# yui-mhcp/text_to_speech

Hardware: AMD Instinct MI355X
Metric: audio samples/sec (22.05 kHz WaveGlow vocoding, fp32) (higher is better)
Workload: dtype f32; 1 GPU; WaveGlow-only vocoding of precomputed 80x800 mel, batch 8 per GPU, fp32 (BASELINE.json configs[1]); batch_per_gpu=8, mel_frames=800, world_size=1, backend=single process, weights=seeded synthetic (rng 1234)

## Files before the change

text_to_speech_amd/csrc/wn_wino.hip:

```cpp
#include "engine.h"
#include "gemm_f32.h"

#include <algorithm>

using namespace ttsgemm;

namespace {
constexpr int C = 512;
constexpr int NPH = 32;
constexpr int KMEL = 320;
constexpr int KCONV = 3 * C;

__device__ __forceinline__ f32x4 x_at(const float* __restrict__ x, int ps, long long f, int df, int c, int PR, int BT, int T) {
    const f32x4 zero = {0.f, 0.f, 0.f, 0.f};
    if (f >= BT) return zero;
    const int carry = (ps >> 5) + df;
    const int t = (int)(f % T) + carry;
    if (t < 0 || t >= T) return zero;
    return *reinterpret_cast<const f32x4*>(x + ((long long)(ps & 31) * PR + f + carry) * C + c);
}


__device__ __forceinline__ int group_phase0(int gp, int d) { return (gp / d) * 4 * d + gp % d; }

__host__ __device__ __forceinline__ int frame_groups_per_utt(int T) { return (T + 15) / 16 * 4; }
__device__ __forceinline__ bool frame_group(int gf, int s, int BT, int T, int& b, int& t0) {
    const int G = frame_groups_per_utt(T);
    b = gf / G;
    const int g = gf % G;
    t0 = (g / s) * 4 * s + g % s;
    return (long long)b * T < BT && t0 < T;
}
__host__ __device__ __forceinline__ int mixed_groups_per_utt(int T) { return (T + 1) / 2; }
__device__ __forceinline__ bool mixed_group(int gm, int BT, int T, int& b, int& t0) {
    const int G = mixed_groups_per_utt(T);
    b = gm / G;
    t0 = 2 * (gm % G);
    return (long long)b * T < BT;
}
__device__ __forceinline__ f32x4 x_bt(const float* __restrict__ x, int p, int b, int t, int c, int PR, int T) {
    const f32x4 zero = {0.f, 0.f, 0.f, 0.f};
    if (t < 0 || t >= T) return zero;
    return *reinterpret_cast<const f32x4*>(x + ((long long)p * PR + (long long)b * T + t) * C + c);
}

__global__ void wino4_prepass_kernel(const float* __restrict__ x, float* __restrict__ U, int d, int PR, int BT, int T, long long Mq) {
    const long long idx = (long long)blockIdx.x * blockDim.x + threadIdx.x;
    if (idx >= Mq * (C / 4)) return;
    const long long mg = idx / (C / 4);
    const int c = (int)(idx % (C / 4)) * 4;
    f32x4 v[6];
    if (d == 16) {
        const int PRm = (int)(Mq / 16);
        const int p0 = (int)(mg / PRm);
        int b, t0;
        const bool ok = mixed_group(mg % PRm, BT, T, b, t0);
        const f32x4 zero = {0.f, 0.f, 0.f, 0.f};
#pragma unroll
        for (int i = 0; i < 6; ++i) {
            const int ps = p0 + 16 * (i - 1);
            v[i] = ok ? x_bt(x, ps & 31, b, t0 + (ps >> 5), c, PR, T) : zero;
        }
    } else if (d < NPH) {
        const int gp = (int)(mg / PR);
        const long long f = mg % PR;
        const int p0 = group_phase0(gp, d);
#pragma unroll
        for (int i = 0; i < 6; ++i) v[i] = x_at(x, p0 + (i - 1) * d, f, 0, c, PR, BT, T);
    } else {
        const int s = d / NPH, PRq = (int)(Mq / NPH);
        const int p = (int)(mg / PRq);
        int b, t0;
        const bool ok = frame_group(mg % PRq, s, BT, T, b, t0);
        const f32x4 zero = {0.f, 0.f, 0.f, 0.f};
#pragma unroll
        for (int i = 0; i < 6; ++i) v[i] = ok ? x_bt(x, p, b, t0 + (i - 1) * s, c, PR, T) : zero;
    }
    const long long o = mg * C + c, plane = Mq * C;
    *reinterpret_cast<f32x4*>(U + o) = 4.f * v[0] - 5.f * v[2] + v[4];
    *reinterpret_cast<f32x4*>(U + plane + o) = -4.f * (v[1] + v[2]) + v[3] + v[4];
    *reinterpret_cast<f32x4*>(U + 2 * plane + o) = 4.f * (v[1] - v[2]) - v[3] + v[4];
    *reinterpret_cast<f32x4*>(U + 3 * plane + o) = 2.f * (v[3] - v[1]) - v[2] + v[4];
    *reinterpret_cast<f32x4*>(U + 4 * plane + o) = 2.f * (v[1] - v[3]) - v[2] + v[4];
    *reinterpret_cast<f32x4*>(U + 5 * plane + o) = 4.f * v[1] - 5.f * v[3] + v[5];
}

__global__ void wino4_weights_kernel(const float* __restrict__ in_Bt, float* __restrict__ G) {
    const int idx = blockIdx.x * blockDim.x + threadIdx.x;
    if (idx >= 2 * C * C) return;
    const int n = idx / C, c = idx % C;
    const float* row = in_Bt + (long long)n * KCONV + (c / 16) * 48 + c % 16;
    const double wm = row[0], w0 = row[16], wp = row[32];
    const long long plane = (long long)2 * C * C;
    G[idx] = (float)(wm / 4.0);
    G[plane + idx] = (float)(-(wm + w0 + wp) / 6.0);
    G[2 * plane + idx] = (float)(-(wm - w0 + wp) / 6.0);
    G[3 * plane + idx] = (float)(wm / 24.0 + w0 / 12.0 + wp / 6.0);
    G[4 * plane + idx] = (float)(wm / 24.0 - w0 / 12.0 + wp / 6.0);
    G[5 * plane + idx] = (float)wp;
}

constexpr int NPT = 7, NMEL = 80;
__constant__ double C44_G[7][4] = {{1., 0., 0., 0.},
                                   {1., 1., 1., 1.},
                                   {1., -1., 1., -1.},
                                   {1., 2., 4., 8.},
                                   {1., -2., 4., -8.},
                                   {1., 1. / 2, 1. / 4, 1. / 8},
                                   {1., -1. / 2, 1. / 4, -1. / 8}};
__constant__ double C44_BT[7][7] = {{1., 0., -21. / 4, 0., 21. / 4, 0., -1.},
                                    {0., -2. / 9, -2. / 9, 17. / 18, 17. / 18, -2. / 9, -2. / 9},
                                    {0., 2. / 9, -2. / 9, -17. / 18, 17. / 18, 2. / 9, -2. / 9},
                                    {0., 1. / 180, 1. / 360, -1. / 36, -1. / 72, 1. / 45, 1. / 90},
                                    {0., -1. / 180, 1. / 360, 1. / 36, -1. / 72, -1. / 45, 1. / 90},
                                    {0., 64. / 45, 128. / 45, -16. / 9, -32. / 9, 16. / 45, 32. / 45},
                                    {0., -64. / 45, 128. / 45, 16. / 9, -32. / 9, -16. / 45, 32. / 45}};

constexpr int K4 = 224, SA = 112, SB = 96, SC = 112;
constexpr int KF = 160;
[[maybe_unused]] __constant__ double FIR_X[5] = {0, 1, -1, 2, -2};
[[maybe_unused]] __constant__ double FIR_BT[5][5] = {{1, 0, -5. / 4, 0, 1. / 4},
                                                     {0, 2. / 3, 2. / 3, -1. / 6, -1. / 6},
                                                     {0, -2. / 3, 2. / 3, 1. / 6, -1. / 6},
                                                     {0, -1. / 12, -1. / 24, 1. / 12, 1. / 24},
                                                     {0, 1. / 12, -1. / 24, -1. / 12, 1. / 24}};
__host__ __device__ __forceinline__ int fir_qb(int s, int half) { return s == 1 ? 2 * half + 1 : half + 2; }
struct InKernelCondChunks {
    unsigned long long cfg_lo = 0, cfg_hi = 0;
};
inline InKernelCondChunks in_kernel_cond_chunks(bool phases, bool mixed, bool fir) {
    InKernelCondChunks a;
    unsigned ccfg[6] = {0, 0, 0, 0, 0, 0};
    auto cc = [](unsigned n1, unsigned b1, unsigned n2 = 0, unsigned b2 = 0) { return n1 | b1 << 5 | n2 << 9 | b2 << 12; };
    if (phases) {
        for (int p = 0; p < 6; ++p) ccfg[p] = cc(p == 1 || p == 2 ? K4 / 16 : (SA + SB) / 16, 0);
    } else if (mixed) {
        for (int p = 1; p < 5; ++p) ccfg[p] = cc(KMEL / 16, 0);
    } else if (fir) {
        for (int p = 0; p < 5; ++p) ccfg[p] = cc(KF / 16, 0);
    } else {
        ccfg[0] = ccfg[5] = cc((SA + SB) / 16, 0);
        ccfg[1] = ccfg[2] = cc(SA / 16, 0, SC / 16, (SA + SB) / 16);
        ccfg[3] = ccfg[4] = cc((SB + SC) / 16, SA / 16);
    }
    for (int p = 0; p < 6; ++p) (p < 4 ? a.cfg_lo : a.cfg_hi) |= (unsigned long long)ccfg[p] << (16 * (p & 3));
    return a;
}

__host__ __device__ __forceinline__ int cond_groups_per_utt(int T) { return (T + 3) / 4; }

__global__ void wino_cond_weights_kernel(const float* __restrict__ cond_Bt, float* __restrict__ W) {
    const long long idx = (long long)blockIdx.x * blockDim.x + threadIdx.x;
    if (idx >= (long long)NPH * NPT * 2 * C * NMEL) return;
    const int c = (int)(idx % NMEL), n = (int)((idx / NMEL) % (2 * C)), x = (int)((idx / ((long long)NMEL * 2 * C)) % NPT),
              p = (int)(idx / ((long long)NMEL * 2 * C * NPT));
    const float* row = cond_Bt + ((long long)p * 2 * C + n) * KMEL + c;
    double acc = 0.0;
#pragma unroll
    for (int q = 0; q < 4; ++q) acc += C44_G[x][3 - q] * (double)row[q * NMEL];
    W[idx] = (float)acc;
}

__global__ void wino_cond_mel_planes_kernel(const float* __restrict__ mel, float* __restrict__ Z, int rows, int BT, int T) {
    const long long idx = (long long)blockIdx.x * blockDim.x + threadIdx.x;
    if (idx >= (long long)NPT * rows * NMEL) return;
    const int c = (int)(idx % NMEL), gr = (int)((idx / NMEL) % rows), x = (int)(idx / ((long long)rows * NMEL));
    const int G = cond_groups_per_utt(T), b = gr / G, t0 = 4 * (gr % G);
    double acc = 0.0;
    if ((long long)b * T < BT) {
#pragma unroll
        for (int i = 0; i < NPT; ++i) {
            const int t = t0 - 3 + i;
            if (t >= 0 && t < T) acc += C44_BT[x][i] * (double)mel[((long long)b * T + t) * NMEL + c];
        }
    }
    Z[idx] = (float)acc;
}

__global__ void wino_cond_rows_kernel(int* __restrict__ tab, int rows, int BT, int T) {
    const int gr = blockIdx.x * blockDim.x + threadIdx.x;
    if (gr >= rows) return;
    const int G = cond_groups_per_utt(T), b = gr / G, t0 = 4 * (gr % G);
    const int left = T - t0;
    tab[gr] = (long long)b * T < BT ? (b * T + t0) | (left < 4 ? left : 4) << 16 : 0;
}

struct WinoCondArgs {
    const float* Z;
    const int* rowtab;
    const float* W;
    const float* bias;
    float* cond;
    int rows;
    int PR, BT, T;
};

template <int WR, int WC, int NBUF, int OCC>
__global__ __launch_bounds__(WR * WC * 64, OCC) void wino_cond_kernel(const WinoCondArgs g) {
    constexpr int NW = WR * WC, BM = WR * 32, BN = WC * 32;
    constexpr int NPA = BM / 16, NPB = BN / 16, PPW = (NPA + NPB) / NW;
    static_assert((NPA + NPB) % NW == 0 && PPW <= 4, "the pieces of a tile divide among the waves, one per MFMA of a half step");
    constexpr int STAGE = (BM + BN) * 16;
    constexpr int NKC = NMEL / 16, NT = NPT * NKC;
    typedef __attribute__((address_space(3))) void* lds_ptr_t;
    extern __shared__ __attribute__((aligned(16))) float smem[];
    const int tid = threadIdx.x, lane = tid & 63;
    const int wave = __builtin_amdgcn_readfirstlane(tid >> 6);
    const int wr = wave / WC, wc = wave % WC;
    const int li = lane & 31, lh = lane >> 5;

    constexpr int numNt = 2 * C / BN;
    const int numMt = g.rows / BM;
    const int bid = blockIdx.x, xcd = bid & 7, slot = bid >> 3;
    const int pair = (slot / numMt) * 8 + xcd, mt = slot % numMt;
    const int ph = pair / numNt, nt = pair % numNt;
    const int m0 = mt * BM, n0 = nt * BN;

    f32x16 acc[NPT];
#pragma unroll
    for (int p = 0; p < NPT; ++p)
#pragma unroll
        for (int r = 0; r < 16; ++r) acc[p][r] = 0.f;

    const int prow = lane >> 2, chunk = (lane & 3) ^ ((lane >> 4) & 3);
    unsigned vo0[PPW];
#pragma unroll
    for (int i = 0; i < PPW; ++i) {
        const int q = wave * PPW + i;
        const int row = (q < NPA ? q : q - NPA) * 16 + prow;
        vo0[i] = (unsigned)((row * NMEL + chunk * 4) * 4);
    }
    const float* const abase = g.Z + (long long)m0 * NMEL;
    const float* const bbase = g.W + ((long long)ph * NPT * 2 * C + n0) * NMEL;
    const long long zplane = (long long)g.rows * NMEL, wplane = (long long)2 * C * NMEL;
    int lt = 0;
    unsigned vo[PPW], ko = 0;
    const float* pb[PPW];
    auto prepare = [&]() {
        const bool live = lt < NT;
        const int x = live ? lt / NKC : 0, kc = live ? lt % NKC : 0;
        ko = (unsigned)kc * 64u;
#pragma unroll
        for (int i = 0; i < PPW; ++i) {
            const bool isA = wave * PPW + i < NPA;
            pb[i] = isA ? abase + x * zplane : bbase + x * wplane;
            vo[i] = live ? vo0[i] : OOB;
        }
        ++lt;
    };
    auto issue_piece = [&](int i, int buf) {
        const unsigned voff = vo[i], koff = ko;
        const float* base = pb[i];
        __builtin_amdgcn_raw_ptr_buffer_load_lds(make_rsrc_uniform(base), (lds_ptr_t)(smem + buf * STAGE + (wave * PPW + i) * 256), 16,
                                                 voff, koff, 0, 0);
    };
    const int xr = (li >> 2) & 3;
    struct Frag {
        f32x4 a, b;
    };
    auto read_frag = [&](int buf, int k8, Frag& f) {
        const int koff = ((2 * k8 + lh) ^ xr) * 4;
        f.a = *reinterpret_cast<const f32x4*>(smem + buf * STAGE + (wr * 32 + li) * 16 + koff);
        f.b = *reinterpret_cast<const f32x4*>(smem + buf * STAGE + BM * 16 + (wc * 32 + li) * 16 + koff);
    };

#pragma unroll
    for (int b = 0; b < NBUF; ++b) {
        prepare();
#pragma unroll
        for (int i = 0; i < PPW; ++i) issue_piece(i, b);
    }
    asm volatile("s_waitcnt vmcnt(%0)" ::"n"(PPW * (NBUF - 1)) : "memory");
    __builtin_amdgcn_s_barrier();
    Frag f0, f1;
    read_frag(0, 0, f0);
    int buf = 0;
    static_for<NPT>([&](auto pc) {
        constexpr int P = decltype(pc)::value;
        for (int s = 0; s < NKC; ++s) {
            read_frag(buf, 1, f1);
            prepare();
#pragma unroll
            for (int kk = 0; kk < 4; ++kk) acc[P] = __builtin_amdgcn_mfma_f32_32x32x2f32(f0.a[kk], f0.b[kk], acc[P], 0, 0, 0);
            __builtin_amdgcn_sched_barrier(0);
            asm volatile("s_waitcnt vmcnt(%0) lgkmcnt(0)" ::"n"(PPW * (NBUF - 2)) : "memory");
            __builtin_amdgcn_s_barrier();
            const int bufn = buf == NBUF - 1 ? 0 : buf + 1;
            read_frag(bufn, 0, f0);
            __builtin_amdgcn_sched_barrier(0);
#pragma unroll
            for (int kk = 0; kk < 4; ++kk) {
                acc[P] = __builtin_amdgcn_mfma_f32_32x32x2f32(f1.a[kk], f1.b[kk], acc[P], 0, 0, 0);
                if (kk < PPW) {
                    issue_piece(kk, buf);
                    __builtin_amdgcn_sched_barrier(0);
                }
            }
            buf = bufn;
        }
    });
    asm volatile("s_waitcnt vmcnt(0)" ::: "memory");

    const float bv = g.bias[n0 + wc * 32 + li];
    const int* const rt = g.rowtab + m0 + wr * 32 + 4 * lh;
    const __amdgpu_buffer_rsrc_t ro = make_rsrc_uniform(g.cond + (long long)ph * g.PR * (2 * C) + n0 + wc * 32);
#pragma unroll
    for (int r = 0; r < 16; ++r) {
        const int info = rt[(r & 3) + 8 * (r >> 2)];
        const unsigned voff = ((unsigned)(info & 0xffff) * (2 * C) + li) * 4u;
        const int nout = info >> 16;
        const float s12 = acc[1][r] + acc[2][r], d12 = acc[1][r] - acc[2][r];
        const float s34 = acc[3][r] + acc[4][r], d34 = acc[3][r] - acc[4][r];
        const float s56 = acc[5][r] + acc[6][r], d56 = acc[5][r] - acc[6][r];
        float y[4];
        y[0] = acc[0][r] + s12 + s34 + s56 + bv;
        y[1] = d12 + 2.f * d34 + 0.5f * d56 + bv;
        y[2] = s12 + 4.f * s34 + 0.25f * s56 + bv;
        y[3] = d12 + 8.f * d34 + 0.125f * d56 + bv;
#pragma unroll
        for (int j = 0; j < 4; ++j)
            __builtin_amdgcn_raw_buffer_store_b32(__builtin_bit_cast(unsigned, y[j]), ro, j < nout ? voff : OOB, j * (2 * C * 4), 0);
    }
}

template <int WR, int WC, int NBUF, int OCC>
hipError_t launch_wino_cond(const WinoCondArgs& a, hipStream_t st) {
    constexpr int BM = WR * 32, BN = WC * 32;
    const size_t lds = (size_t)NBUF * (BM + BN) * 16 * sizeof(float);
    if (a.rows % BM != 0) return hipErrorInvalidValue;
    auto kern = wino_cond_kernel<WR, WC, NBUF, OCC>;
    static PerDeviceOnce attr_set;
    if (hipError_t e = set_max_dyn_lds_once((const void*)kern, lds, attr_set); e != hipSuccess) return e;
    hipLaunchKernelGGL(kern, dim3((unsigned)(NPH * (2 * C / BN) * (a.rows / BM))), dim3(WR * WC * 64), lds, st, a);
    return hipGetLastError();
}

__device__ __forceinline__ unsigned group_out_pack(int kind, int gl, int sfr, int BT, int T) {
    if (kind == 0) return (unsigned)gl | 15u << 20;
    int b, t0;
    const bool ok = kind == 1 ? frame_group(gl, sfr, BT, T, b, t0) : mixed_group(gl, BT, T, b, t0);
    if (!ok) return 0u;
    const int left = T - t0;
    return (unsigned)(b * T + t0) | (unsigned)(left < 15 ? left : 15) << 20;
}
__device__ __forceinline__ long long group_out_base(int kind, int ph, int j, int d, int PR, unsigned& jstep) {
    if (kind == 0) {
        jstep = 0;
        return (long long)(group_phase0(ph, d) + j * d) * PR;
    }
    if (kind == 1) {
        jstep = (unsigned)(j * (d / NPH));
        return (long long)ph * PR + j * (d / NPH);
    }
    jstep = (unsigned)(j >> 1);
    return (long long)(ph + 16 * (j & 1)) * PR + (j >> 1);
}

__global__ void wino4_combine_kernel(const float* __restrict__ P, const float* __restrict__ cond, float* __restrict__ acts, int d,
                                     int PR, int BT, int T, long long Mq) {
    const long long idx = (long long)blockIdx.x * blockDim.x + threadIdx.x;
    if (idx >= Mq * (C / 4)) return;
    const long long mg = idx / (C / 4);
    const int ch = (int)(idx % (C / 4)) * 4;
    const int col = (ch >> 5) * 64 + (ch & 31);
    const long long plane = Mq * 2 * C, o = mg * 2 * C + col;
    f32x4 a[6], b[6];
#pragma unroll
    for (int z = 0; z < 6; ++z) {
        a[z] = __builtin_nontemporal_load(reinterpret_cast<const f32x4*>(P + z * plane + o));
        b[z] = __builtin_nontemporal_load(reinterpret_cast<const f32x4*>(P + z * plane + o + 32));
    }
    const int kind = d == 16 ? 2 : d < NPH ? 0 : 1;
    const int prows = kind == 0 ? PR : (int)(Mq / (kind == 2 ? 16 : NPH));
    const int ph = (int)(mg / prows);
    const unsigned pack = group_out_pack(kind, (int)(mg % prows), d / NPH, BT, T);
#pragma unroll
    for (int j = 0; j < 4; ++j) {
        unsigned jstep;
        const long long row = group_out_base(kind, ph, j, d, PR, jstep) + (pack & 0xfffffu);
        if (jstep >= pack >> 20) break;
        const f32x4 ca = *reinterpret_cast<const f32x4*>(cond + row * (2 * C) + col);
        const f32x4 cb = *reinterpret_cast<const f32x4*>(cond + row * (2 * C) + col + 32);
        f32x4 t, s;
        if (j == 0) {
            t = a[0] + a[1] + a[2] + a[3] + a[4] + ca;
            s = b[0] + b[1] + b[2] + b[3] + b[4] + cb;
        } else if (j == 1) {
            t = a[1] - a[2] + 2.f * (a[3] - a[4]) + ca;
            s = b[1] - b[2] + 2.f * (b[3] - b[4]) + cb;
        } else if (j == 2) {
            t = a[1] + a[2] + 4.f * (a[3] + a[4]) + ca;
            s = b[1] + b[2] + 4.f * (b[3] + b[4]) + cb;
        } else {
            t = a[1] - a[2] + 8.f * (a[3] - a[4]) + a[5] + ca;
            s = b[1] - b[2] + 8.f * (b[3] - b[4]) + b[5] + cb;
        }
        f32x4 g;
#pragma unroll
        for (int k = 0; k < 4; ++k) g[k] = gate_tanh_sigmoid(t[k], s[k]);
        *reinterpret_cast<f32x4*>(acts + row * C + ch) = g;
    }
}

__device__ __forceinline__ void wino_gate_store(const f32x16 (&acc)[6][2], float* patch, const float* __restrict__ cond,
                                                float* __restrict__ acts, int kind, int d, int ph, int gl0, int col0, int PR, int BT,
                                                int T, int lane) {
    const int li = lane & 31, lh = lane >> 5, er = lane >> 3, ec4 = (lane & 7) * 4;
    const int sfr = d / NPH;
    const int ch0 = (col0 >> 6) * 32 + ec4;
    unsigned orow[16];
#pragma unroll
    for (int r = 0; r < 16; ++r) {
        orow[r] = group_out_pack(kind, gl0 + (r & 3) + 8 * (r >> 2) + 4 * lh, sfr, BT, T);
        __builtin_amdgcn_sched_barrier(0);
    }
    static_for<4>([&](auto jc) {
        constexpr int j = decltype(jc)::value;
        unsigned jstep;
        const long long jb = group_out_base(kind, ph, j, d, PR, jstep);
        const __amdgpu_buffer_rsrc_t rc = make_rsrc_uniform(cond + jb * (2 * C) + col0);
        constexpr int RB = j == 0 ? 8 : 16;
#pragma unroll
        for (int r0 = 0; r0 < 16; r0 += RB) {
            float ctv[RB], csv[RB];
#pragma unroll
            for (int rr = 0; rr < RB; ++rr) {
                const unsigned pk = orow[r0 + rr];
                const unsigned off = jstep < pk >> 20 ? ((pk & 0xfffffu) * (2 * C) + li) * 4u : OOB;
                ctv[rr] = __builtin_bit_cast(float, __builtin_amdgcn_raw_buffer_load_b32(rc, off, 0, 0));
                csv[rr] = __builtin_bit_cast(float, __builtin_amdgcn_raw_buffer_load_b32(rc, off, 128, 0));
            }
            __builtin_amdgcn_sched_barrier(0);
#pragma unroll
            for (int rr = 0; rr < RB; ++rr) {
                const int r = r0 + rr;
                const float ct = ctv[rr], cs = csv[rr];
                float tv, sv;
                if constexpr (j == 0) {
                    tv = acc[0][0][r] + acc[1][0][r] + acc[2][0][r] + acc[3][0][r] + acc[4][0][r] + ct;
                    sv = acc[0][1][r] + acc[1][1][r] + acc[2][1][r] + acc[3][1][r] + acc[4][1][r] + cs;
                } else if constexpr (j == 1) {
                    tv = acc[1][0][r] - acc[2][0][r] + 2.f * (acc[3][0][r] - acc[4][0][r]) + ct;
                    sv = acc[1][1][r] - acc[2][1][r] + 2.f * (acc[3][1][r] - acc[4][1][r]) + cs;
                } else if constexpr (j == 2) {
                    tv = acc[1][0][r] + acc[2][0][r] + 4.f * (acc[3][0][r] + acc[4][0][r]) + ct;
                    sv = acc[1][1][r] + acc[2][1][r] + 4.f * (acc[3][1][r] + acc[4][1][r]) + cs;
                } else {
                    tv = acc[1][0][r] - acc[2][0][r] + 8.f * (acc[3][0][r] - acc[4][0][r]) + acc[5][0][r] + ct;
                    sv = acc[1][1][r] - acc[2][1][r] + 8.f * (acc[3][1][r] - acc[4][1][r]) + acc[5][1][r] + cs;
                }
                patch[((r & 3) + 8 * (r >> 2) + 4 * lh) * 36 + li] = gate_tanh_sigmoid(tv, sv);
            }
        }
        asm volatile("s_waitcnt lgkmcnt(0)" ::: "memory");
#pragma unroll
        for (int qq = 0; qq < 4; ++qq) {
            const f32x4 v = *reinterpret_cast<const f32x4*>(patch + (er + 8 * qq) * 36 + ec4);
            const unsigned srow = group_out_pack(kind, gl0 + er + 8 * qq, sfr, BT, T);
            if (jstep < srow >> 20) *reinterpret_cast<f32x4*>(acts + (jb + (srow & 0xfffffu)) * C + ch0) = v;
        }
        asm volatile("s_waitcnt lgkmcnt(0)" ::: "memory");
    });
}

struct WinoFusedArgs {
    const float* U;   long long uplane;
    const float* G;   long long gplane;
    const float* cond;
    float* acts;
    int Mq, phase_rows;
    int kind;
    int d, PR, BT, T;
};

template <int WR, int WC, int NBUF, int OCC>
__global__ __launch_bounds__(WR * WC * 64, OCC) void wino4_fused_kernel(const WinoFusedArgs g) {
    constexpr int NW = WR * WC, BM = WR * 32, BN = WC * 64;
    constexpr int NPA = BM / 16, NPB = BN / 16, PPW = (NPA + NPB) / NW;
    static_assert((NPA + NPB) % NW == 0, "the pieces of a tile divide among the waves");
    constexpr int STAGE = (BM + BN) * 16;
    static_assert(NBUF * STAGE >= NW * 32 * 36, "the epilogue's transpose patches fit the pipeline buffers");
    typedef __attribute__((address_space(3))) void* lds_ptr_t;
    extern __shared__ __attribute__((aligned(16))) float smem[];
    const int tid = threadIdx.x, lane = tid & 63;
    const int wave = __builtin_amdgcn_readfirstlane(tid >> 6);
    const int wr = wave / WC, wc = wave % WC;
    const int li = lane & 31, lh = lane >> 5;

    constexpr int numNt = 2 * C / BN;
    const int numMt = g.Mq / BM;
    const int bid = blockIdx.x, xcd = bid & 7, slot = bid >> 3;
    const int mt = (slot / numNt) * 8 + xcd, nt = slot % numNt;
    if (mt >= numMt) return;
    const int m0 = mt * BM, n0 = nt * BN;
    const int ph = m0 / g.phase_rows, fr0 = m0 - ph * g.phase_rows;

    f32x16 acc[6][2];
#pragma unroll
    for (int p = 0; p < 6; ++p)
#pragma unroll
        for (int h = 0; h < 2; ++h)
#pragma unroll
            for (int r = 0; r < 16; ++r) acc[p][h][r] = 0.f;

    const int prow = lane >> 2, chunk = (lane & 3) ^ ((lane >> 4) & 3);
    unsigned vo0[PPW];
#pragma unroll
    for (int i = 0; i < PPW; ++i) {
        const int q = wave * PPW + i;
        const int row = (q < NPA ? q : q - NPA) * 16 + prow;
        vo0[i] = (unsigned)((row * C + chunk * 4) * 4);
    }
    int lp = 0, lkc = 0;
    unsigned vo[PPW], ko = 0;
    const float* pb[PPW];
    auto prepare = [&]() {
        const bool live = lp < 6;
        const int p = live ? lp : 0;
        ko = (unsigned)lkc * 64u;
#pragma unroll
        for (int i = 0; i < PPW; ++i) {
            const bool isA = wave * PPW + i < NPA;
            pb[i] = isA ? g.U + p * g.uplane + (long long)m0 * C : g.G + p * g.gplane + (long long)n0 * C;
            vo[i] = live ? vo0[i] : OOB;
        }
        if (live && ++lkc == C / 16) {
            lkc = 0;
            ++lp;
        }
    };
    auto issue_piece = [&](int i, int buf) {
        const unsigned voff = vo[i], koff = ko;
        const float* base = pb[i];
        __builtin_amdgcn_raw_ptr_buffer_load_lds(make_rsrc_uniform(base), (lds_ptr_t)(smem + buf * STAGE + (wave * PPW + i) * 256), 16,
                                                 voff, koff, 0, 0);
    };
    const int xr = (li >> 2) & 3;
    struct Frag {
        f32x4 a, b0, b1;
    };
    auto read_frag = [&](int buf, int k8, Frag& f) {
        const int koff = ((2 * k8 + lh) ^ xr) * 4;
        const float* a = smem + buf * STAGE + (wr * 32 + li) * 16 + koff;
        const float* b = smem + buf * STAGE + BM * 16 + (wc * 64 + li) * 16 + koff;
        f.a = *reinterpret_cast<const f32x4*>(a);
        f.b0 = *reinterpret_cast<const f32x4*>(b);
        f.b1 = *reinterpret_cast<const f32x4*>(b + 32 * 16);
    };

#pragma unroll
    for (int b = 0; b < NBUF; ++b) {
        prepare();
#pragma unroll
        for (int i = 0; i < PPW; ++i) issue_piece(i, b);
    }
    asm volatile("s_waitcnt vmcnt(%0)" ::"n"(PPW * (NBUF - 1)) : "memory");
    __builtin_amdgcn_s_barrier();
    Frag f0, f1;
    read_frag(0, 0, f0);
    int buf = 0;
    static_for<6>([&](auto pc) {
        constexpr int P = decltype(pc)::value;
        for (int s = 0; s < C / 16; ++s) {
            read_frag(buf, 1, f1);
            prepare();
#pragma unroll
            for (int kk = 0; kk < 4; ++kk) {
                acc[P][0] = __builtin_amdgcn_mfma_f32_32x32x2f32(f0.a[kk], f0.b0[kk], acc[P][0], 0, 0, 0);
                acc[P][1] = __builtin_amdgcn_mfma_f32_32x32x2f32(f0.a[kk], f0.b1[kk], acc[P][1], 0, 0, 0);
            }
            __builtin_amdgcn_sched_barrier(0);
            asm volatile("s_waitcnt vmcnt(%0) lgkmcnt(0)" ::"n"(PPW * (NBUF - 2)) : "memory");
            __builtin_amdgcn_s_barrier();
            const int bufn = buf == NBUF - 1 ? 0 : buf + 1;
            read_frag(bufn, 0, f0);
            __builtin_amdgcn_sched_barrier(0);
#pragma unroll
            for (int kk = 0; kk < 4; ++kk) {
                acc[P][0] = __builtin_amdgcn_mfma_f32_32x32x2f32(f1.a[kk], f1.b0[kk], acc[P][0], 0, 0, 0);
                acc[P][1] = __builtin_amdgcn_mfma_f32_32x32x2f32(f1.a[kk], f1.b1[kk], acc[P][1], 0, 0, 0);
                if (kk < PPW) {
                    issue_piece(kk, buf);
                    __builtin_amdgcn_sched_barrier(0);
                }
            }
            static_assert(PPW <= 4, "one DMA piece per MFMA pair of the second half");
            buf = bufn;
        }
    });
    asm volatile("s_waitcnt vmcnt(0)" ::: "memory");
    __builtin_amdgcn_s_barrier();

    wino_gate_store(acc, smem + wave * (32 * 36), g.cond, g.acts, g.kind, g.d, ph, fr0 + wr * 32, n0 + wc * 64, g.PR, g.BT, g.T, lane);
}

template <int WR, int WC, int NBUF, int OCC>
hipError_t launch_wino_fused(const WinoFusedArgs& a, hipStream_t st) {
    constexpr int BM = WR * 32, BN = WC * 64;
    const size_t lds = (size_t)NBUF * (BM + BN) * 16 * sizeof(float);
    if (a.Mq % BM != 0 || a.phase_rows % BM != 0 || a.Mq % a.phase_rows != 0) return hipErrorInvalidValue;
    auto kern = wino4_fused_kernel<WR, WC, NBUF, OCC>;
    static PerDeviceOnce attr_set;
    if (hipError_t e = set_max_dyn_lds_once((const void*)kern, lds, attr_set); e != hipSuccess) return e;
    const int numMt8 = (a.Mq / BM + 7) / 8 * 8;
    hipLaunchKernelGGL(kern, dim3(numMt8 * (2 * C / BN)), dim3(WR * WC * 64), lds, st, a);
    return hipGetLastError();
}

struct WinoFused2Args {
    const float* x;
    const float* G;   long long gplane;
    const float* cond;
    float* acts;
    int Mq, phase_rows, kind, d, PR, BT, T;
};

__global__ __launch_bounds__(256, 2) void wino4_fused2_kernel(const WinoFused2Args g) {
    constexpr int BM = 64, BN = 128, NBUF = 3, NG = C / 16;
    constexpr int XT = BM * 16, XS = 6 * XT, BS = BN * 16;
    typedef __attribute__((address_space(3))) void* lds_ptr_t;
    extern __shared__ __attribute__((aligned(16))) float smem[];
    float* const xs = smem;
    float* const Bs = smem + 2 * XS;
    const int tid = threadIdx.x, lane = tid & 63;
    const int wave = __builtin_amdgcn_readfirstlane(tid >> 6);
    const int wr = wave >> 1, wc = wave & 1;
    const int li = lane & 31, lh = lane >> 5;

    constexpr int numNt = 2 * C / BN;
    const int numMt = g.Mq / BM;
    const int bid = blockIdx.x, xcd = bid & 7, slot = bid >> 3;
    const int mt = (slot / numNt) * 8 + xcd, nt = slot % numNt;
    if (mt >= numMt) return;
    const int m0 = mt * BM, n0 = nt * BN;
    const int ph = m0 / g.phase_rows, fr0 = m0 - ph * g.phase_rows;

    f32x16 acc[6][2];
#pragma unroll
    for (int p = 0; p < 6; ++p)
#pragma unroll
        for (int h = 0; h < 2; ++h)
#pragma unroll
            for (int r = 0; r < 16; ++r) acc[p][h][r] = 0.f;

    const int prow = lane >> 2, chunk = (lane & 3) ^ ((lane >> 4) & 3);
    const int sfr = g.d / NPH;
    unsigned xbase = 0, xvalid = 0;
    int xdelta[6];
    {
        const int gl = fr0 + wave * 16 + prow;
        int b = 0, t0 = 0;
        bool ok;
        if (g.kind == 0) {
            ok = gl < g.BT;
            t0 = gl % g.T;
            xbase = (unsigned)gl;
        } else if (g.kind == 1) {
            ok = frame_group(gl, sfr, g.BT, g.T, b, t0);
            xbase = (unsigned)(b * g.T + t0);
        } else {
            ok = mixed_group(gl, g.BT, g.T, b, t0);
            xbase = (unsigned)(b * g.T + t0);
        }
#pragma unroll
        for (int i = 0; i < 6; ++i) {
            int dt;
            if (g.kind == 0) {
                const int ps = group_phase0(ph, g.d) + (i - 1) * g.d;
                dt = ps >> 5;
                xdelta[i] = ((ps & 31) * g.PR + dt) * C;
            } else if (g.kind == 1) {
                dt = (i - 1) * sfr;
                xdelta[i] = (ph * g.PR + dt) * C;
            } else {
                const int ps = ph + 16 * (i - 1);
                dt = ps >> 5;
                xdelta[i] = ((ps & 31) * g.PR + dt) * C;
            }
            if (ok && t0 + dt >= 0 && t0 + dt < g.T) xvalid |= 1u << i;
        }
        xbase = xbase * (unsigned)(C * 4) + (unsigned)chunk * 16u;
    }
    const unsigned vb0 = (unsigned)(((2 * wave * 16 + prow) * C + chunk * 4) * 4);

    const float* const gb0 = g.G + (long long)n0 * C;
    auto issue_x = [&](auto ic, int grp) {
        constexpr int I = decltype(ic)::value;
        const unsigned voff = (grp < NG && ((xvalid >> I) & 1u)) ? xbase : OOB;
        const float* base = g.x + (long long)xdelta[I];
        __builtin_amdgcn_raw_ptr_buffer_load_lds(make_rsrc_uniform(base), (lds_ptr_t)(xs + (grp & 1) * XS + I * XT + wave * 256), 16, voff,
                                                 (unsigned)grp * 64u, 0, 0);
    };
    auto issue_b_taps = [&](int j, int prod, int grp, int buf) {
        const float* base = gb0 + prod * (2 * C * C);
        const unsigned voff = grp < NG ? vb0 : OOB;
        __builtin_amdgcn_raw_ptr_buffer_load_lds(make_rsrc_uniform(base), (lds_ptr_t)(Bs + buf * BS + (2 * wave + j) * 256), 16, voff,
                                                 (unsigned)grp * 64u + (unsigned)j * (16u * C * 4u), 0, 0);
    };
    const int xr = (li >> 2) & 3;
    struct Frag {
        f32x4 a, b0, b1;
    };
    struct Raw {
        f32x4 v[4];
    };
    auto read_b = [&](int buf, int h, Frag& f) {
        const float* b = Bs + buf * BS + (wc * 64 + li) * 16 + ((2 * h + lh) ^ xr) * 4;
        f.b0 = *reinterpret_cast<const f32x4*>(b);
        f.b1 = *reinterpret_cast<const f32x4*>(b + 32 * 16);
    };
    auto read_x = [&](auto pc, int stage, int h, Raw& r) {
        constexpr int P = decltype(pc)::value;
        const float* a = xs + stage * XS + (wr * 32 + li) * 16 + ((2 * h + lh) ^ xr) * 4;
        constexpr int i0 = P == 0 ? 0 : 1, i1 = P == 0 ? 2 : P == 5 ? 3 : 2, i2 = P == 0 ? 4 : P == 5 ? 5 : 3;
        r.v[0] = *reinterpret_cast<const f32x4*>(a + i0 * XT);
        r.v[1] = *reinterpret_cast<const f32x4*>(a + i1 * XT);
        r.v[2] = *reinterpret_cast<const f32x4*>(a + i2 * XT);
        if constexpr (P >= 1 && P <= 4) r.v[3] = *reinterpret_cast<const f32x4*>(a + 4 * XT);
    };
    auto combine = [&](auto pc, const Raw& r) -> f32x4 {
        constexpr int P = decltype(pc)::value;
        if constexpr (P == 0) return 4.f * r.v[0] - 5.f * r.v[1] + r.v[2];
        else if constexpr (P == 1) return -4.f * (r.v[0] + r.v[1]) + r.v[2] + r.v[3];
        else if constexpr (P == 2) return 4.f * (r.v[0] - r.v[1]) - r.v[2] + r.v[3];
        else if constexpr (P == 3) return 2.f * (r.v[2] - r.v[0]) - r.v[1] + r.v[3];
        else if constexpr (P == 4) return 2.f * (r.v[0] - r.v[2]) - r.v[1] + r.v[3];
        else return 4.f * r.v[0] - 5.f * r.v[1] + r.v[2];
    };
    auto mfma2 = [&](auto pc, const Frag& f, int kk) {
        constexpr int P = decltype(pc)::value;
        acc[P][0] = __builtin_amdgcn_mfma_f32_32x32x2f32(f.a[kk], f.b0[kk], acc[P][0], 0, 0, 0);
        acc[P][1] = __builtin_amdgcn_mfma_f32_32x32x2f32(f.a[kk], f.b1[kk], acc[P][1], 0, 0, 0);
    };

    static_for<5>([&](auto ic) { issue_x(ic, 0); });
    issue_b_taps(0, 0, 0, 0); issue_b_taps(1, 0, 0, 0);
    issue_b_taps(0, 1, 0, 1); issue_b_taps(1, 1, 0, 1);
    issue_x(std::integral_constant<int, 5>{}, 0);
    issue_b_taps(0, 2, 0, 2); issue_b_taps(1, 2, 0, 2);
    asm volatile("s_waitcnt vmcnt(5)" ::: "memory");
    __builtin_amdgcn_s_barrier();
    Frag f0, f1;
    Raw raw;
    read_x(std::integral_constant<int, 0>{}, 0, 0, raw);
    read_b(0, 0, f0);
    f0.a = combine(std::integral_constant<int, 0>{}, raw);

    int buf = 0;
    for (int grp = 0; grp < NG; ++grp) {
        const int stage = grp & 1;
        static_for<6>([&](auto pc) {
            constexpr int P = decltype(pc)::value;
            constexpr int PN = (P + 1) % 6, P3 = (P + 3) % 6;
            constexpr int XI = P < 3 ? 2 * P : P == 3 ? 1 : P == 4 ? 3 : 5;
            read_x(pc, stage, 1, raw);
            mfma2(pc, f0, 0);
            mfma2(pc, f0, 1);
            __builtin_amdgcn_sched_barrier(0);
            f1.a = combine(pc, raw);
            read_b(buf, 1, f1);
            __builtin_amdgcn_sched_barrier(0);
            mfma2(pc, f0, 2);
            mfma2(pc, f0, 3);
            __builtin_amdgcn_sched_barrier(0);
            asm volatile("s_waitcnt vmcnt(3) lgkmcnt(0)" ::: "memory");
            __builtin_amdgcn_s_barrier();
            const int bufn = buf == NBUF - 1 ? 0 : buf + 1;
            read_x(std::integral_constant<int, PN>{}, P == 5 ? stage ^ 1 : stage, 0, raw);
            __builtin_amdgcn_sched_barrier(0);
            mfma2(pc, f1, 0);
            issue_x(std::integral_constant<int, XI>{}, grp + 1);
            __builtin_amdgcn_sched_barrier(0);
            mfma2(pc, f1, 1);
            __builtin_amdgcn_sched_barrier(0);
            f0.a = combine(std::integral_constant<int, PN>{}, raw);
            read_b(bufn, 0, f0);
            __builtin_amdgcn_sched_barrier(0);
            mfma2(pc, f1, 2);
            issue_b_taps(0, P3, grp + (P >= 3 ? 1 : 0), buf);
            __builtin_amdgcn_sched_barrier(0);
            mfma2(pc, f1, 3);
            issue_b_taps(1, P3, grp + (P >= 3 ? 1 : 0), buf);
            __builtin_amdgcn_sched_barrier(0);
            buf = bufn;
        });
    }
    asm volatile("s_waitcnt vmcnt(0)" ::: "memory");
    __builtin_amdgcn_s_barrier();

    wino_gate_store(acc, smem + wave * (32 * 36), g.cond, g.acts, g.kind, g.d, ph, fr0 + wr * 32, n0 + wc * 64, g.PR, g.BT, g.T, lane);
}

hipError_t launch_wino_fused2(const WinoFused2Args& a, hipStream_t st) {
    constexpr int BM = 64, BN = 128;
    const size_t lds = (size_t)(2 * 6 * BM * 16 + 3 * BN * 16) * sizeof(float);
    if (a.Mq % BM != 0 || a.phase_rows % BM != 0 || a.Mq % a.phase_rows != 0) return hipErrorInvalidValue;
    static PerDeviceOnce attr_set;
    if (hipError_t e = set_max_dyn_lds_once((const void*)wino4_fused2_kernel, lds, attr_set); e != hipSuccess) return e;
    const int numMt8 = (a.Mq / BM + 7) / 8 * 8;
    hipLaunchKernelGGL(wino4_fused2_kernel, dim3(numMt8 * (2 * C / BN)), dim3(256), lds, st, a);
    return hipGetLastError();
}

inline unsigned blocks_for(long long n) { return (unsigned)((n + 255) / 256); }
}

static inline int group_row_tile(int form) { return form == 2 ? 128 : 64; }
static inline int frame_group_rows(int BT, int T, int form) {
    const int g = group_row_tile(form);
    return ((BT / T) * frame_groups_per_utt(T) + g - 1) / g * g;
}
static inline int mixed_group_rows(int BT, int T, int form) {
    const int g = group_row_tile(form);
    return ((BT / T) * mixed_groups_per_utt(T) + g - 1) / g * g;
}

static inline int cond_group_rows(int BT, int T) { return ((BT / T) * cond_groups_per_utt(T) + 63) / 64 * 64; }

int waveglow_build_wino(tts_hip_engine* e) {
    WaveGlowDev& wg = e->wg;
    if (wg.wino_ready) return TTS_HIP_OK;
    hipStream_t st = e->stream;
    std::vector<void*> fresh;
    auto fail = [&](int rc) {
        (void)hipStreamSynchronize(st);
        for (void* p : fresh) (void)hipFree(p);
        for (int k = 0; k < 12; ++k)
            for (int i = 1; i < 8; ++i) wg.flow[k].layer[i].wino_G = wg.flow[k].layer[i].wino_W = nullptr;
        return rc;
    };
    for (int k = 0; k < 12; ++k)
        for (int i = 1; i < 8; ++i) {
            WgLayerDev& ly = wg.flow[k].layer[i];
            const long long nw = (long long)NPH * NPT * 2 * C * NMEL;
            int rc;
            if ((rc = dev_alloc(e, (size_t)6 * 2 * C * C, &ly.wino_G, fresh, false))) return fail(rc);
            hipLaunchKernelGGL(wino4_weights_kernel, dim3(blocks_for(2 * C * C)), dim3(256), 0, st, ly.in_Bt, ly.wino_G);
            if ((rc = dev_alloc(e, (size_t)nw, &ly.wino_W, fresh, false))) return fail(rc);
            hipLaunchKernelGGL(wino_cond_weights_kernel, dim3(blocks_for(nw)), dim3(256), 0, st, ly.cond_Bt, ly.wino_W);
            if (hipError_t herr = hipGetLastError(); herr != hipSuccess)
                return fail(set_err(e, TTS_HIP_EHIP, "waveglow_build_wino: %s", hipGetErrorString(herr)));
        }
    if (hipError_t herr = hipStreamSynchronize(st); herr != hipSuccess)
        return fail(set_err(e, TTS_HIP_EHIP, "waveglow_build_wino: %s", hipGetErrorString(herr)));
    wg.allocs.insert(wg.allocs.end(), fresh.begin(), fresh.end());
    wg.wino_ready = true;
    return TTS_HIP_OK;
}

int waveglow_wino_begin(tts_hip_engine* e, const float* d_mel, int PR, int BT, int T, int form) {
    const bool three_pass = form == 2, need_U = form != 1;
    WaveGlowDev& wg = e->wg;
    hipStream_t st = e->stream;
    const int PRq = frame_group_rows(BT, T, form), PRm = mixed_group_rows(BT, T, form), PRc = cond_group_rows(BT, T);
    const size_t rows = 6 * (size_t)std::max(std::max((long long)(NPH / 4) * PR, (long long)NPH * PRq), (long long)16 * PRm);
    auto room = [&](DevBuf& b, size_t bytes) -> int {
        const hipError_t err = b.ensure(bytes);
        if (err == hipSuccess) return TTS_HIP_OK;
        if (err == hipErrorOutOfMemory) (void)hipGetLastError();
        return set_err(e, err == hipErrorOutOfMemory ? TTS_HIP_ENOMEM : TTS_HIP_EHIP, "waveglow_wino_begin: hipMalloc(%zu bytes) -> %s",
                       bytes, hipGetErrorString(err));
    };
    int rc;
    if (need_U && (rc = room(wg.wino_U, rows * C * 4))) return rc;
    if (three_pass && (rc = room(wg.wino_P, rows * 2 * C * 4))) return rc;
    if ((rc = room(wg.wino_mel, ((size_t)NPT * PRc * NMEL + PRc) * 4))) return rc;
    const size_t before = wg.wino_cond.bytes;
    if ((rc = room(wg.wino_cond, (size_t)NPH * PR * 2 * C * 4))) return rc;
    if (wg.wino_cond.bytes != before) HIPCHK(e, hipMemsetAsync(wg.wino_cond.p, 0, wg.wino_cond.bytes, st));
    hipLaunchKernelGGL(wino_cond_mel_planes_kernel, dim3(blocks_for((long long)NPT * PRc * NMEL)), dim3(256), 0, st, d_mel,
                       wg.wino_mel.f(), PRc, BT, T);
    hipLaunchKernelGGL(wino_cond_rows_kernel, dim3(blocks_for(PRc)), dim3(256), 0, st, (int*)(wg.wino_mel.f() + (size_t)NPT * PRc * NMEL),
                       PRc, BT, T);
    HIPCHK(e, hipGetLastError());
    return TTS_HIP_OK;
}

int waveglow_wino_layer(tts_hip_engine* e, const WgLayerDev& ly, int i, const float* x, float* acts_i, int PR, int BT, int T) {
    WaveGlowDev& wg = e->wg;
    hipStream_t st = e->stream;
    const int d = 1 << i;
    float* U = wg.wino_U.f();
    float* P = wg.wino_P.f();
    const int PRq = frame_group_rows(BT, T, wg.form_mode), PRm = mixed_group_rows(BT, T, wg.form_mode);
    const bool phases = d <= 8, mixed = d == 16;
    const long long Mq = phases ? (long long)(NPH / 4) * PR : mixed ? (long long)16 * PRm : (long long)NPH * PRq;
    WinoCondArgs c{};
    c.Z = wg.wino_mel.f();
    c.W = ly.wino_W;
    c.bias = ly.in_bias;
    c.cond = wg.wino_cond.f();
    c.rows = cond_group_rows(BT, T);
    c.rowtab = (const int*)(c.Z + (size_t)NPT * c.rows * NMEL);
    c.PR = PR;
    c.BT = BT;
    c.T = T;
    const bool no_prepass = wg.form_mode == 1;
    if (!no_prepass) hipLaunchKernelGGL(wino4_prepass_kernel, dim3(blocks_for(Mq * (C / 4))), dim3(256), 0, st, x, U, d, PR, BT, T, Mq);
    if (wg.form_mode != 2) {
        WinoFusedArgs a{};
        a.U = U;
        a.uplane = Mq * C;
        a.G = ly.wino_G;
        a.gplane = (long long)2 * C * C;
        a.cond = c.cond;
        a.acts = acts_i;
        a.Mq = (int)Mq;
        a.phase_rows = phases ? PR : mixed ? PRm : PRq;
        a.kind = phases ? 0 : mixed ? 2 : 1;
        a.d = d;
        a.PR = PR;
        a.BT = BT;
        a.T = T;
        if (no_prepass) {
            WinoFused2Args b{};
            b.x = x;
            b.G = a.G; b.gplane = a.gplane;
            b.cond = a.cond; b.acts = a.acts;
            b.Mq = a.Mq; b.phase_rows = a.phase_rows; b.kind = a.kind; b.d = a.d; b.PR = a.PR; b.BT = a.BT; b.T = a.T;
            timing_begin(e, 0);
            HIPCHK(e, (launch_wino_cond<2, 2, 3, 3>(c, st)));
            HIPCHK(e, launch_wino_fused2(b, st));
            timing_end(e);
            return TTS_HIP_OK;
        }
        timing_begin(e, 0);
        HIPCHK(e, (launch_wino_cond<2, 2, 3, 3>(c, st)));
        HIPCHK(e, (launch_wino_fused<2, 2, 3, 2>(a, st)));
        timing_end(e);
        return TTS_HIP_OK;
    }
    GemmArgs g{};
    g.M = (int)Mq;
    g.N = 2 * C;
    g.nphase = phases ? NPH / 4 : mixed ? 16 : NPH;
    g.phase_rows = phases ? PR : mixed ? PRm : PRq;
    g.frames = phases ? BT : mixed ? (BT / T) * mixed_groups_per_utt(T) : (BT / T) * frame_groups_per_utt(T);
    g.L = g.phase_rows;
    g.ldb = C;
    g.mode = EPI_LINEAR;
    g.act = ACT_NONE;
    g.split = 2 * C;
    g.ld0 = 2 * C;
    g.wide_epi = 1;
    g.nseg = 1;
    g.seg[0] = ASeg{U, C, 0, C, C, SEG_ROWS_Z, 0, Mq, 0};
    g.Bt = ly.wino_G;
    g.strideBz = (long long)2 * C * C;
    g.out0 = P;
    g.strideOutZ = Mq * 2 * C;
    timing_begin(e, 0);
    HIPCHK(e, (launch_wino_cond<2, 2, 3, 3>(c, st)));
    HIPCHK(e, phases && PR % 256 == 0 ? gemm_wn_wino(g, 6, st) : gemm_wn_wino_128(g, 6, st));
    timing_end(e);
    hipLaunchKernelGGL(wino4_combine_kernel, dim3(blocks_for(Mq * (C / 4))), dim3(256), 0, st, P, c.cond, acts_i, d, PR, BT, T, Mq);
    HIPCHK(e, hipGetLastError());
    return TTS_HIP_OK;
}
```

Baseline: 4.326 million audio samples/s.

## Prefetch conditioning into LDS via buffer DMA in Winograd gate epilogue

Replaces the fused Winograd kernel's gate/store epilogue with a version that loads the conditioning tiles straight into LDS using buffer_load_lds. These loads are double-buffered across the four output phases, so the next phase's conditioning is in flight while the current phase is gated. Stores go out through buffer_store_b128 with out-of-range masking, over a swizzled 32x64 staging layout that should avoid bank conflicts. Optional timestamp instrumentation is also added behind a compile flag; it is off by default. The new epilogue uses more LDS per wave for the two staging tiles, and the hand-tuned vmcnt wait counts must match the number of loads actually issued.

```diff
diff --git a/text_to_speech_amd/csrc/wn_wino.hip b/text_to_speech_amd/csrc/wn_wino.hip
--- a/text_to_speech_amd/csrc/wn_wino.hip
+++ b/text_to_speech_amd/csrc/wn_wino.hip
@@ -463,6 +463,98 @@
     });
 }
 
+__host__ __device__ constexpr int wino_stage_row(int k, int lane) { return 4 * k + (lane >> 4); }
+__host__ __device__ constexpr int wino_stage_piece(int lane) { return (lane & 15) ^ (((lane >> 5) & 1) << 3); }
+__host__ __device__ constexpr int wino_stage_at(int row, int col) { return row * 64 + (col ^ (((row >> 1) & 1) << 5)); }
+
+__device__ __forceinline__ void wino_gate_store_dma(const f32x16 (&acc)[6][2], float* stage, const float* __restrict__ cond,
+                                                    float* __restrict__ acts, int kind, int d, int ph, int gl0, int col0, int PR,
+                                                    int BT, int T, int lane) {
+    typedef __attribute__((address_space(3))) void* lds_ptr_t;
+    constexpr int TILE = 32 * 64;
+    const int li = lane & 31, lh = lane >> 5, er = lane >> 3, ec4 = (lane & 7) * 4;
+    const int sfr = d / NPH;
+    unsigned drow[8], srow[4];
+#pragma unroll
+    for (int k = 0; k < 8; ++k) {
+        drow[k] = group_out_pack(kind, gl0 + wino_stage_row(k, lane), sfr, BT, T);
+        __builtin_amdgcn_sched_barrier(0);
+    }
+#pragma unroll
+    for (int qq = 0; qq < 4; ++qq) {
+        srow[qq] = group_out_pack(kind, gl0 + er + 8 * qq, sfr, BT, T);
+        __builtin_amdgcn_sched_barrier(0);
+    }
+    const unsigned dcol = (unsigned)wino_stage_piece(lane) * 16u;
+    auto request = [&](auto jc) {
+        constexpr int J = decltype(jc)::value;
+        unsigned jstep;
+        const long long jb = group_out_base(kind, ph, J, d, PR, jstep);
+        const __amdgpu_buffer_rsrc_t rc = make_rsrc_uniform(cond + jb * (2 * C) + col0);
+#pragma unroll
+        for (int k = 0; k < 8; ++k) {
+            const unsigned pk = drow[k];
+            const unsigned voff = jstep < pk >> 20 ? (pk & 0xfffffu) * (2 * C * 4) + dcol : OOB;
+            __builtin_amdgcn_raw_ptr_buffer_load_lds(rc, (lds_ptr_t)(stage + (J & 1) * TILE + k * 256), 16, voff, 0, 0, 0);
+        }
+    };
+    request(std::integral_constant<int, 0>{});
+    request(std::integral_constant<int, 1>{});
+    static_for<4>([&](auto jc) {
+        constexpr int j = decltype(jc)::value;
+        unsigned jstep;
+        const long long jb = group_out_base(kind, ph, j, d, PR, jstep);
+        float* const mine = stage + (j & 1) * TILE + lh * (4 * 64) + li;
+        asm volatile("s_waitcnt vmcnt(%0)" ::"n"(j == 0 ? 8 : j == 1 ? 12 : j == 2 ? 16 : 8) : "memory");
+        constexpr int RB = j == 0 ? 8 : 16;
+#pragma unroll
+        for (int r0 = 0; r0 < 16; r0 += RB) {
+            float ctv[RB], csv[RB];
+#pragma unroll
+            for (int rr = 0; rr < RB; ++rr) {
+                const int r = r0 + rr, row = (r & 3) + 8 * (r >> 2);
+                ctv[rr] = mine[wino_stage_at(row, 0)];
+                csv[rr] = mine[wino_stage_at(row, 32)];
+            }
+            __builtin_amdgcn_sched_barrier(0);
+#pragma unroll
+            for (int rr = 0; rr < RB; ++rr) {
+                const int r = r0 + rr;
+                const float ct = ctv[rr], cs = csv[rr];
+                float tv, sv;
+                if constexpr (j == 0) {
+                    tv = acc[0][0][r] + acc[1][0][r] + acc[2][0][r] + acc[3][0][r] + acc[4][0][r] + ct;
+                    sv = acc[0][1][r] + acc[1][1][r] + acc[2][1][r] + acc[3][1][r] + acc[4][1][r] + cs;
+                } else if constexpr (j == 1) {
+                    tv = acc[1][0][r] - acc[2][0][r] + 2.f * (acc[3][0][r] - acc[4][0][r]) + ct;
+                    sv = acc[1][1][r] - acc[2][1][r] + 2.f * (acc[3][1][r] - acc[4][1][r]) + cs;
+                } else if constexpr (j == 2) {
+                    tv = acc[1][0][r] + acc[2][0][r] + 4.f * (acc[3][0][r] + acc[4][0][r]) + ct;
+                    sv = acc[1][1][r] + acc[2][1][r] + 4.f * (acc[3][1][r] + acc[4][1][r]) + cs;
+                } else {
+                    tv = acc[1][0][r] - acc[2][0][r] + 8.f * (acc[3][0][r] - acc[4][0][r]) + acc[5][0][r] + ct;
+                    sv = acc[1][1][r] - acc[2][1][r] + 8.f * (acc[3][1][r] - acc[4][1][r]) + acc[5][1][r] + cs;
+                }
+                mine[wino_stage_at((r & 3) + 8 * (r >> 2), 0)] = gate_tanh_sigmoid(tv, sv);
+            }
+        }
+        asm volatile("s_waitcnt lgkmcnt(0)" ::: "memory");
+        f32x4 v[4];
+#pragma unroll
+        for (int qq = 0; qq < 4; ++qq)
+            v[qq] = *reinterpret_cast<const f32x4*>(stage + (j & 1) * TILE + (er + 8 * qq) * 64 + (((er >> 1) & 1) << 5) + ec4);
+        asm volatile("s_waitcnt lgkmcnt(0)" ::: "memory");
+        if constexpr (j + 2 < 4) request(std::integral_constant<int, j + 2>{});
+        const __amdgpu_buffer_rsrc_t ra = make_rsrc_uniform(acts + jb * C + (col0 >> 6) * 32);
+#pragma unroll
+        for (int qq = 0; qq < 4; ++qq) {
+            const unsigned pk = srow[qq];
+            const unsigned voff = jstep < pk >> 20 ? (pk & 0xfffffu) * (C * 4) + (unsigned)ec4 * 4u : OOB;
+            __builtin_amdgcn_raw_buffer_store_b128(__builtin_bit_cast(u32x4, v[qq]), ra, voff, 0, 0);
+        }
+    });
+}
+
 struct WinoFusedArgs {
     const float* U;   long long uplane;
     const float* G;   long long gplane;
@@ -615,6 +707,16 @@
     int Mq, phase_rows, kind, d, PR, BT, T;
 };
 
+#ifdef TTS_WINO_STAMPS
+__device__ unsigned long long g_wino_stamps[4 * 8192];
+#define WINO_STAMP(i)                                                                               \
+    do {                                                                                            \
+        if (tid == 0 && bid < 8192) g_wino_stamps[4 * bid + (i)] = __builtin_amdgcn_s_memtime();    \
+    } while (0)
+#else
+#define WINO_STAMP(i) do { } while (0)
+#endif
+
 __global__ __launch_bounds__(256, 2) void wino4_fused2_kernel(const WinoFused2Args g) {
     constexpr int BM = 64, BN = 128, NBUF = 3, NG = C / 16;
     constexpr int XT = BM * 16, XS = 6 * XT, BS = BN * 16;
@@ -634,6 +736,12 @@
     if (mt >= numMt) return;
     const int m0 = mt * BM, n0 = nt * BN;
     const int ph = m0 / g.phase_rows, fr0 = m0 - ph * g.phase_rows;
+#ifdef TTS_WINO_STAMPS
+    if (tid == 0 && bid < 8192)
+        g_wino_stamps[4 * bid + 3] = (unsigned long long)__builtin_amdgcn_s_getreg(31 << 11 | 4) |
+                                     (unsigned long long)__builtin_amdgcn_s_getreg(31 << 11 | 20) << 32;
+#endif
+    WINO_STAMP(0);
 
     f32x16 acc[6][2];
 #pragma unroll
@@ -787,8 +895,11 @@
     }
     asm volatile("s_waitcnt vmcnt(0)" ::: "memory");
     __builtin_amdgcn_s_barrier();
-
-    wino_gate_store(acc, smem + wave * (32 * 36), g.cond, g.acts, g.kind, g.d, ph, fr0 + wr * 32, n0 + wc * 64, g.PR, g.BT, g.T, lane);
+    WINO_STAMP(1);
+
+    wino_gate_store_dma(acc, smem + wave * (2 * 32 * 64), g.cond, g.acts, g.kind, g.d, ph, fr0 + wr * 32, n0 + wc * 64, g.PR, g.BT, g.T,
+                        lane);
+    WINO_STAMP(2);
 }
 
 hipError_t launch_wino_fused2(const WinoFused2Args& a, hipStream_t st) {
@@ -801,6 +912,15 @@
     hipLaunchKernelGGL(wino4_fused2_kernel, dim3(numMt8 * (2 * C / BN)), dim3(256), lds, st, a);
     return hipGetLastError();
 }
+
+#ifdef TTS_WINO_STAMPS
+}
+extern "C" __attribute__((visibility("default"))) int tts_hip_debug_wino_stamps(unsigned long long* out, int n) {
+    if (n < 0 || n > 8192 || hipDeviceSynchronize() != hipSuccess) return -1;
+    return hipMemcpyFromSymbol(out, HIP_SYMBOL(g_wino_stamps), (size_t)n * 4 * sizeof(unsigned long long)) == hipSuccess ? 0 : -1;
+}
+namespace {
+#endif
 
 inline unsigned blocks_for(long long n) { return (unsigned)((n + 255) / 256); }
 }
```

Result: faster. 4.413 million audio samples/s (median of 6 runs) (+2.0%).
